# JunkyByte/easy_ViTPose

Measured on AMD Instinct MI355X. Metric: persons_per_sec, higher is better.
Workload: dtype fp16; 1 GPU; ViTPose-B coco K=17, batch 256 x 256x192 crops per GPU (f32 input resident in HBM) -> (y,x,conf) keypoints in HBM; global_batch=256, weights=seeded random init (no checkpoint offline)

## Files before the change

easy_vitpose_amd/build.py:

```python
from __future__ import annotations

import os
import shutil
import subprocess
import sys
from concurrent.futures import ThreadPoolExecutor

HERE = os.path.dirname(os.path.abspath(__file__))
CSRC = os.path.join(HERE, 'csrc')
LIBDIR = os.path.join(HERE, '_lib')
LIB = os.path.join(LIBDIR, 'libvitpose_hip.so')
TOOLS_LIB = os.path.join(LIBDIR, 'libvitpose_hip_tools.so')
SOURCES = ['gemm.hip', 'gemm8.hip', 'gemm8f.hip', 'qkvattn.hip', 'quant8.hip', 'attention.hip', 'elementwise.hip', 'decode.hip', 'boxes.hip', 'fp8_probe.hip',
           'handle.hip', 'forward.hip', 'infer.hip', 'group.hip', 'weights.hip', 'tile_rules.hip', 'debug_taps.hip']
TOOLS_SOURCES = SOURCES + ['probes.hip', 'tools_taps.hip']
HEADERS = ['common.h', 'kernels.h', 'tiles.h', 'dbg_util.h', 'gemm8_common.h', 'mx8.h', 'api_internal.h', 'boxgeom.h', os.path.join('..', '..', 'include', 'vitpose_hip.h'),
           os.path.join('..', '..', 'include', 'vitpose_hip_tools.h')]
FLAGS = ['--offload-arch=gfx950', '-O3', '-std=c++17', '-fPIC', '-fvisibility=hidden',
         '-ffp-contract=fast', '-Wno-unused-result']


def _hipcc() -> str:
    for cand in (shutil.which('hipcc'), '/opt/rocm/bin/hipcc'):
        if cand and os.path.exists(cand):
            return cand
    raise RuntimeError('hipcc not found: the HIP extension cannot be built (no CPU fallback exists)')


def _stale(target: str, deps: "list[str]") -> bool:
    if not os.path.exists(target):
        return True
    t = os.path.getmtime(target)
    return any(os.path.getmtime(d) > t for d in deps)


def build_library(force: bool = False, verbose: bool = False, tools: bool = False) -> str:
    os.makedirs(LIBDIR, exist_ok=True)
    hipcc = _hipcc()
    hdrs = [os.path.normpath(os.path.join(CSRC, h)) for h in HEADERS]
# ... 30 lines not shown
```

easy_vitpose_amd/csrc/api_internal.h:

```cpp
#pragma once
#include <hip/hip_runtime.h>

#include <algorithm>
#include <cmath>
#include <cstdio>
#include <cstdlib>
#include <cstring>
#include <string>
#include <unordered_map>
#include <vector>

#include "../../include/vitpose_hip.h"
#ifdef VP_TOOLS
#include "../../include/vitpose_hip_tools.h"
#endif
#include "kernels.h"
#include "mx8.h"

namespace vpi {

struct Block {
    float *ln1_g, *ln1_b, *ln2_g, *ln2_b;
    uint16_t *w_qkv, *w_proj, *w_fc1, *w_fc2;
    float *b_qkv, *b_proj, *b_fc1, *b_fc2;
    float *s_qkv, *s_fc1;
    uint16_t* w_qkvh = nullptr;
    float *b_qkvh = nullptr, *s_qkvh = nullptr;
    uint8_t *w_qkv8 = nullptr, *w_fc18 = nullptr, *w_fc28 = nullptr, *w_proj8 = nullptr;
    float *ws_qkv = nullptr, *ws_fc1 = nullptr, *ws_fc2 = nullptr, *ws_proj = nullptr;
};

struct Switches {
    int g8_stagger = 0;
    int gemm8_mask = 0x7;
    long g8_min_tiles = 448;
    bool persist_gemm = true;
    int order_mask = 8;
    bool blocked_hid = true;
    bool blocked_qkv = true;
    bool fuse_ln = true;
    bool fuse_qkv_attn = true;
    bool qa_min_set = false;
    long qa_min_tiles = 108;
    long qa80_min_tiles = 192;
    int qa80_group = 8;
    int attn_qsplit = 128;
    int g8_bm192 = 3;
    bool pad_batch = true;
    bool g8_cost_model = true;
    bool deconv_parity_fast = true;
    bool fuse_head = true;
    bool fp8_proj16 = false;
    int graph_max_n = 16;
    bool graph_null = true;
    int caller_stream_max_n = 16;
    bool fold_rule = true;
    int graph_max_n_stats = 8;
    bool splitk_on = true;
    int splitk_force[2][2] = {{0, 0}, {0, 0}};
    int gemm_variant[VP_PROF_COUNT] = {-1, -1, -1, -1, -1, -1, -1, -1, -1, -1, -1};
    int gemm_group_m[VP_PROF_COUNT] = {0};
    int fam_ablate[VP_PROF_COUNT] = {0};
};

}

namespace vpi {
struct MixPlan {
// ... 191 lines not shown
    size_t plane = 0;
    float* stats_out = nullptr;
    const float* rowstat = nullptr;
    const float* ln_s = nullptr;
    const float* ln_part = nullptr;
    int ln_tiles = 0;
    int* tiles_out = nullptr;
};

constexpr int SPLITK_MAX_S = 8, SPLITK_MAX_CROPS = 32;
struct GemmPick { int variant = -1, group_m = 0, persist = 0, stagger = 0, splitk = 1, splitk_variant = 0; };
GemmPick resolve_gemm(const Switches& s, int fam, int epi, int M, int N, int K, bool ln_part = false, size_t splitk_rows = 0,
                      const std::vector<int>* mix_bounds = nullptr);
GemmPick resolve_gemm_fp8(int fam, int epi, int Mp, int N);
enum QkvPath { QKV_GEMM = 0, QKV_ATTN64 = 1, QKV_ATTN80 = 2 };
struct HeadPlan {
    bool fused = false;
    GemmPick deconv1, deconv2, final;
};
struct ChunkPlan {
    int n = 0;
    bool fold1 = false, fold2 = false;
    int qkv_path = QKV_GEMM;
    bool attn_qsplit = false;
    bool proj_fp8 = false;
    GemmPick gemm[VP_PROF_COUNT];
    HeadPlan head;
};
ChunkPlan plan_chunk(const Switches& s, int D, int heads, int max_batch, bool fp8, int n_in, size_t fin_rows, const std::vector<int>* mix_bounds = nullptr);
HeadPlan plan_head(const Switches& s, int D, int nh, size_t fin_rows);

int gemm(vp_ctx* c, int fam, int epi, const GemmPick& pk, const uint16_t* A, const uint16_t* W, const float* bias, void* out,
         const float* aux, int M, int N, int K, int ldo, int Hin = 0, int Win = 0, int Cin = 0, const LnFuse* ln = nullptr);
int gemm_fp8(vp_ctx* c, int fam, int epi, const GemmPick& pk, const uint8_t* A8, const uint8_t* a_scales, const uint8_t* W8, const float* w_scale, const float* bias,
             void* out, uint8_t* out_scales, const float* aux, int M, int N, int K, const LnFuse* ln);
struct FwdOpts {
    bool tokens = false;
    bool mirror = false;
    bool head = true;
    int twin_src = 0;
};
int forward_chunk(vp_ctx* c, const void* d_crops, int fmt, int n_in, const FwdOpts& o = FwdOpts());
int head_chunk(vp_ctx* c, const uint16_t* y, int nh, float* hm, const HeadPlan& hp);
int decode_chunk(vp_ctx* c, const int32_t* d_wh, float* d_out, int n, bool twin);
int chunk_cap(const vp_ctx* c);
int chunk_rows(const vp_ctx* c, int nb);
// ... 5 lines not shown
```

easy_vitpose_amd/csrc/forward.hip:

```cpp
#include "api_internal.h"
#include "tiles.h"

using namespace vpi;

namespace vpi {

static void note_kernel(vp_ctx* c, int fam, const char* desc) {
    if (desc[0] && c->kernel_desc[fam] != desc) c->kernel_desc[fam] = desc;
}

int gemm(vp_ctx* c, int fam, int epi, const GemmPick& pk, const uint16_t* A, const uint16_t* W, const float* bias, void* out,
         const float* aux, int M, int N, int K, int ldo, int Hin, int Win, int Cin, const LnFuse* ln) {
    vp::GemmArgs g{};
    g.A = A; g.W = W; g.bias = bias; g.out = out; g.aux = aux;
    g.M = M; g.N = N; g.K = K; g.ldo = ldo;
    g.Hin = Hin; g.Win = Win; g.Cin = Cin; g.zero = c->zero; g.Kp = c->Kp;
    g.w_rows = (int)pad128((size_t)N);
    g.variant = pk.variant; g.group_m = pk.group_m; g.persist = pk.persist; g.stagger = pk.stagger;
    g.ablate = c->gemm_ablate | c->sw.fam_ablate[fam];
    g.parity_fast = c->sw.deconv_parity_fast;
    if (c->mix_expert && fam == VP_PROF_GEMM_FC2) g.expert = c->mix_expert;
    if (ln) {
        g.a_blocked = ln->a_blocked; g.out_blocked = ln->out_blocked; g.reverse = ln->reverse;
        g.plane = ln->plane; g.stats_out = ln->stats_out; g.rowstat = ln->rowstat; g.ln_s = ln->ln_s;
// ... 126 lines not shown
        };
        const double qkv_attn_flops = 2.0 * M * 3.0 * D * D + 4.0 * 192 * 192 * (double)D * n, qkv_attn_bytes = 2.0 * M * D + 2.0 * 3 * D * (double)D + 2.0 * M * D;
        if ((rc = gemm(c, VP_PROF_GEMM_PATCH, vp::EPI_POS_LN, pk[VP_PROF_GEMM_PATCH], c->hid, c->w_patch, c->b_zero, c->x, c->pos, M, D, 768, D, 0, 0, 0, &prod))) return rc;
        if ((rc = finalize(pl.fold1))) return rc;
        for (int l = 0; l < c->L; ++l) {
            const Block& b = c->blocks[l];
            if (pl.qkv_path == QKV_ATTN80) {
                vp::GemmArgs g80{};
                g80.A = xh; g80.W = b.w_qkvh; g80.bias = b.b_qkvh; g80.ln_s = b.s_qkvh; g80.rowstat = c->rowstat; g80.out = c->y;
                g80.M = M; g80.N = c->heads * 256; g80.K = D; g80.ldo = D; g80.w_rows = c->heads * 256; g80.variant = 18;
                g80.group_m = c->sw.qa80_group;
                g80.attn_scale_log2e = (1.0f / sqrtf(80.0f)) * 1.4426950408889634f;
                g80.ablate = c->gemm_ablate | c->sw.fam_ablate[VP_PROF_GEMM_QKV];
                char desc[192];
                desc[0] = 0;
                g80.desc = desc; g80.desc_cap = (int)sizeof(desc);
                LAUNCH(c, VP_PROF_GEMM_QKV, qkv_attn_flops, qkv_attn_bytes, vp::gemm_launch(c->dtype, vp::EPI_QKV_ATTN, g80, c->stream));
                note_kernel(c, VP_PROF_GEMM_QKV, desc);
            } else if (pl.qkv_path == QKV_ATTN64) {
                vp::QkvAttnArgs qa{};
                qa.x_hi = xh; qa.wh = b.w_qkvh; qa.bh = b.b_qkvh; qa.sh = b.s_qkvh; qa.rowstat = c->rowstat; qa.y = c->y;
                qa.npairs = (n + 1) / 2; qa.ncrops = n; qa.heads = c->heads; qa.D = D;
                qa.scale_log2e = (1.0f / sqrtf(64.0f)) * 1.4426950408889634f;
                char desc[96];
                desc[0] = 0;
                LAUNCH(c, VP_PROF_GEMM_QKV, qkv_attn_flops, qkv_attn_bytes, vp::qkvattn_launch(c->dtype, qa, c->stream, desc, (int)sizeof(desc)));
                note_kernel(c, VP_PROF_GEMM_QKV, desc);
            } else {
                LnFuse cq; cq.rowstat = c->rowstat; cq.ln_s = b.s_qkv; cq.reverse = (c->sw.order_mask & 1) != 0; cq.out_blocked = qkv_blocked;
                if (pl.fold1) { cq.rowstat = nullptr; cq.ln_part = c->ln_part; cq.ln_tiles = D / 64; }
                if ((rc = gemm(c, VP_PROF_GEMM_QKV, vp::EPI_BIAS, pk[VP_PROF_GEMM_QKV], xh, b.w_qkv, b.b_qkv, c->qkv, nullptr, M, 3 * D, D, 3 * D, 0, 0, 0, &cq))) return rc;
                if ((rc = attention(c->y, 8.0 * M * D, nullptr))) return rc;
            }
            LnFuse pp = prod; pp.reverse = (c->sw.order_mask & 2) != 0;
            if ((rc = gemm(c, VP_PROF_GEMM_PROJ, vp::EPI_BIAS_RESID_LN, pk[VP_PROF_GEMM_PROJ], c->y, b.w_proj, b.b_proj, c->x, c->x, M, D, D, D, 0, 0, 0, &pp))) return rc;
            if ((rc = finalize(pl.fold2))) return rc;
            LnFuse c1; c1.rowstat = c->rowstat; c1.ln_s = b.s_fc1; c1.out_blocked = c->sw.blocked_hid; c1.reverse = (c->sw.order_mask & 4) != 0;
            if (pl.fold2) { c1.rowstat = nullptr; c1.ln_part = c->ln_part; c1.ln_tiles = D / 64; }
            if ((rc = gemm(c, VP_PROF_GEMM_FC1, vp::EPI_BIAS_GELU, pk[VP_PROF_GEMM_FC1], xh, b.w_fc1, b.b_fc1, c->hid, nullptr, M, 4 * D, D, 4 * D, 0, 0, 0, &c1))) return rc;
            LnFuse p2 = prod; p2.a_blocked = c->sw.blocked_hid; p2.reverse = (c->sw.order_mask & 8) != 0;
            if ((rc = gemm(c, VP_PROF_GEMM_FC2, vp::EPI_BIAS_RESID_LN, pk[VP_PROF_GEMM_FC2], c->hid, fc2_w(c, b), fc2_b(c, b), c->x, c->x, M, D, 4 * D, D, 0, 0, 0, &p2))) return rc;
            if (l + 1 < c->L && (rc = finalize(pl.fold1))) return rc;
        }
    } else {
    if ((rc = gemm(c, VP_PROF_GEMM_PATCH, vp::EPI_POS, pk[VP_PROF_GEMM_PATCH], c->hid, c->w_patch, c->b_zero, c->x, c->pos, M, D, 768, D))) return rc;
    for (int l = 0; l < c->L; ++l) {
// ... 178 lines not shown
```

easy_vitpose_amd/csrc/handle.hip:

```cpp
#include "api_internal.h"

using namespace vpi;

namespace vpi {

thread_local std::string g_create_error;

int fail(vp_ctx* c, int code, const std::string& msg) {
    if (c) c->err = msg; else g_create_error = msg;
    return code;
}

int need_weights(vp_ctx* c) {
    if (!c) return VP_ERR_INVALID;
    return c->loaded ? (int)VP_OK : fail(c, VP_ERR_STATE, "weights not loaded: call vp_load_weights first");
}

bool slots_busy(const vp_ctx* c) { return c->slots[0].busy || c->slots[1].busy; }

int slots_idle(vp_ctx* c, const char* who) {
    return slots_busy(c) ? fail(c, VP_ERR_STATE, std::string(who) + " with a vp_infer_submit in flight: call vp_infer_wait first") : (int)VP_OK;
}

int quiesce(vp_ctx* c) {
// ... 44 lines not shown
            t += used;
            if (*t == ',') ++t; else break;
        }
    }
#endif
}

void read_switches(Switches& s) {
    auto on = [](const char* name, bool& dst) { if (const char* f = getenv(name)) dst = atoi(f) != 0; };
    auto num = [](const char* name, auto& dst) { if (const char* f = getenv(name)) dst = atol(f); };
    on("VP_FUSE_LN", s.fuse_ln);
    on("VP_PERSIST", s.persist_gemm);
    if (const char* f = getenv("VP_GRAPH")) s.graph_max_n = atoi(f) == 1 ? 16 : atoi(f);
    on("VP_GRAPH_NULL", s.graph_null);
    if (const char* f = getenv("VP_CALLER_STREAM")) s.caller_stream_max_n = atoi(f) == 1 ? 16 : atoi(f);
    on("VP_FUSE_HEAD", s.fuse_head);
    if (const char* f = getenv("VP_FOLD_STATS")) { s.graph_max_n_stats = atoi(f); s.fold_rule = false; }
    on("VP_BLOCKED_QKV", s.blocked_qkv);
    on("VP_FUSE_QKV_ATTN", s.fuse_qkv_attn);
    s.qa_min_set = getenv("VP_QA_MIN_TILES") != nullptr;
    num("VP_QA_MIN_TILES", s.qa_min_tiles);
    num("VP_QA80_MIN_TILES", s.qa80_min_tiles);
    num("VP_QA80_GROUP", s.qa80_group);
    num("VP_ATTN_QSPLIT", s.attn_qsplit);
    on("VP_DECONV_PARITY_FAST", s.deconv_parity_fast);
    on("VP_G8_COST", s.g8_cost_model);
    on("VP_PAD_BATCH", s.pad_batch);
    num("VP_G8_BM192", s.g8_bm192);
    if (const char* f = getenv("VP_SPLITK")) {
        if (!strchr(f, ':')) s.splitk_on = atoi(f) != 0;
        else {
            const char* t = f;
            while (*t) {
                const int which = !strncmp(t, "fc2:", 4) ? 1 : !strncmp(t, "proj:", 5) ? 0 : -1;
                if (which < 0) break;
                t = strchr(t, ':') + 1;
                int S = 0, v = 0, used = 0;
                if (sscanf(t, "%d:%d%n", &S, &v, &used) != 2) break;
                s.splitk_force[which][0] = S; s.splitk_force[which][1] = v;
                t += used;
                if (*t == ',') ++t;
            }
        }
    }
    num("VP_GEMM8", s.gemm8_mask);
    s.fp8_proj16 = getenv("VP_FP8_PROJ16") != nullptr;
// ... 287 lines not shown
```

easy_vitpose_amd/csrc/kernels.h:

```cpp
#pragma once
#include <hip/hip_runtime.h>
#include <stdint.h>

#ifdef VP_TOOLS
#define VP_ABLATE(g) ((g).ablate)
#define VP_STAGGER(g) ((g).stagger)
namespace vp {
hipError_t peak_bench(int kind, double* result);
hipError_t hwid_probe_launch(uint32_t* d_out, int blocks, int threads, int lds_bytes, int spin, hipStream_t s);
}
#else
#define VP_ABLATE(g) 0
#define VP_STAGGER(g) 0
#endif

namespace vp {

enum { DT_F16 = 0, DT_BF16 = 1 };

enum GemmEpi {
    EPI_BIAS = 0,
    EPI_BIAS_GELU = 1,
    EPI_BIAS_RESID = 2,
    EPI_POS = 3,
    EPI_DECONV = 4,
// ... 63 lines not shown
hipError_t ln_finalize_launch(const float* partials, float* rowstat, int M, int tiles, int D, hipStream_t s);
hipError_t splitk_reduce_launch(int dtype, const float* partials, int S, const float* bias, uint16_t* x_hi, size_t plane, float* stats_out, int M, int N,
                                hipStream_t s);

hipError_t fp8_probe_launch(const float* dA, const float* dW, const float* dAs, const float* dWs, uint8_t* dA8, uint8_t* dW8, float* dOut,
                            int M, int N, int K, hipStream_t s);

hipError_t mx_probe_launch(const float* dA, const float* dW, const float* dWs, uint8_t* dA8, uint8_t* dAs, uint8_t* dW8, float* dOut,
                           int M, int N, int K, hipStream_t s);

hipError_t attention_launch(int dtype, const uint16_t* qkv, uint16_t* out, int B, int D, int heads, hipStream_t s, bool qsplit, int qkv_blocked = 0,
                            uint8_t* mx_scales = nullptr);

struct QkvAttnArgs {
    const uint16_t* x_hi;
    const uint16_t* wh;
    const float* bh;
    const float* sh;
    const float* rowstat;
    uint16_t* y;
    int npairs, heads, D;
    int ncrops;
    float scale_log2e;
    int ablate;
};
bool qkvattn_supported(const QkvAttnArgs& a);
hipError_t qkvattn_launch(int dtype, const QkvAttnArgs& a, hipStream_t s, char* desc, int desc_cap);
hipError_t qkv_head_major_launch(const uint16_t* w, const float* b, const float* s, uint16_t* wh, float* bh, float* sh, int D, int K, hipStream_t st);
hipError_t qkv_head_major80_launch(const uint16_t* w, const float* b, const float* s, uint16_t* wh, float* bh, float* sh, int D, int K, int heads, hipStream_t st);

hipError_t layernorm_launch(int dtype, const float* x, const float* gamma, const float* beta,
                            uint16_t* out16, float* out32, int M, int D, hipStream_t s, size_t plane = 0);
hipError_t im2col_launch(int dtype, const void* crops, int input_format, uint16_t* out, int B, hipStream_t s, bool flip = false, int n_src = 0);
hipError_t gather_crops_launch(const void* src, void* dst, const int32_t* idx, int n, size_t crop_bytes, hipStream_t s);
hipError_t flip_merge_launch(float* hm, const float* hm_flipped, const int32_t* partner, int N, int K, int shift, hipStream_t s, int interleaved = 0);
hipError_t im2col_twin_launch(int dtype, const void* crops, int input_format, uint16_t* out, int B, int n_src, hipStream_t s);
void flip_twin_layout(int bo, int n_src, int* src, int* mirror);

struct CropRec {
    const uint8_t* src;
    int64_t pitch;
    int32_t cw, ch, left, top, pw, ph;
};
hipError_t crop_resize_launch(const CropRec* recs, uint8_t* out, int n, hipStream_t s);

constexpr int BOX_FRAMES_PER_LAUNCH = 128;
// ... 32 lines not shown
```

easy_vitpose_amd/csrc/qkvattn.hip:

```cpp
#include <cstdio>
#include <cstdlib>

#include "gemm8_common.h"

namespace vp {

namespace {
struct QA {
    static constexpr int NT = 512;
    static constexpr int XS = 192 * 128;
    static constexpr int W0S = 128 * 128, W1S = 64 * 128;
    static constexpr int OFF_X0 = 0, OFF_X1 = XS, OFF_W0 = 2 * XS, OFF_W1 = 2 * XS + W0S;
    static constexpr int BUF = 2 * XS + W0S + W1S;
    static constexpr int RING = 2 * BUF;
    static constexpr int VSUB = 192 * 32;
    static constexpr int V_BASE = 4 * XS;
    static_assert(6 * XS == RING && BUF <= 3 * XS && BUF + XS <= 4 * XS, "the attention phase reuses exactly the ring; buffer 0 + X0 of buffer 1 inside Q0 K0 Q1 K1");
};

__device__ __forceinline__ u32x2 lds_read_tr16(const char* p) {
    typedef __attribute__((__vector_size__(4 * sizeof(__fp16)))) __fp16 h4;
    typedef __attribute__((address_space(3))) h4* lds_h4;
    const h4 v = __builtin_amdgcn_ds_read_tr16_b64_v4f16((lds_h4)(p));
    return __builtin_bit_cast(u32x2, v);
}
}

template <class T>
__global__ __launch_bounds__(512, 2) void qkvattn_kernel(QkvAttnArgs g) {
    constexpr int QT = 3;
    extern __shared__ __attribute__((aligned(16))) char smem[];
    const int tid = threadIdx.x, lane = tid & 63;
    const int wave = __builtin_amdgcn_readfirstlane(tid >> 6);
    const int wr = wave >> 2, wc = wave & 3;
    const int K = g.D, nk = K >> 6;
    const int ntiles = g.npairs * g.heads;
    const int xcd = blockIdx.x & 7, j0 = blockIdx.x >> 3;
    const int nloc = (gridDim.x >> 3) + (xcd < (int)(gridDim.x & 7) ? 1 : 0);
    const int tq = ntiles >> 3, tr8 = ntiles & 7;
    const int tbase = (xcd < tr8) ? xcd * (tq + 1) : tr8 * (tq + 1) + (xcd - tr8) * tq;
    const int tcnt = tq + (xcd < tr8 ? 1 : 0);
    if (j0 >= tcnt) return;

    const int rip = lane >> 3, pslot = lane & 7;
    const int slog = pslot ^ (((wave & 1) << 2) | (rip >> 1));
    const uint32_t voff = (uint32_t)(rip * K + slog * 8) * 2u;
    const size_t r64 = (size_t)64 * K * 2;
    const char* xb = nullptr;
    const char* wb = nullptr;
    size_t xb1off = 0;
    int pair = 0, head = 0;
    int ipair = 0, ihead = 0;
    auto set_tile = [&](int t) {
        const int tile = tbase + t;
        ipair = tile / g.heads;
        ihead = tile - ipair * g.heads;
        xb = (const char*)(g.x_hi + ((size_t)ipair * 384 + wave * 8) * K);
        xb1off = (2 * ipair + 1 < g.ncrops) ? (size_t)192 * K * 2 : 0;
        wb = (const char*)(g.wh + ((size_t)ihead * 192 + wave * 8) * K);
    };
    auto issue = [&](int which, int B, int kt) {
        char* dst = smem + B * QA::BUF + wave * 1024;
        uint32_t v = voff;
        asm volatile("" : "+v"(v));
        if (which < 2) {
            const char* src = xb + (which ? xb1off : 0) + (size_t)kt * 128 + v;
            glds16(src, dst + which * QA::XS);
            glds16(src + r64, dst + which * QA::XS + 8192);
            glds16(src + 2 * r64, dst + which * QA::XS + 16384);
        } else if (which == 2) {
            const char* src = wb + (size_t)kt * 128 + v;
            glds16(src, dst + QA::OFF_W0);
            glds16(src + r64, dst + QA::OFF_W0 + 8192);
        } else {
            const char* src = wb + 2 * r64 + (size_t)kt * 128 + v;
            glds16(src, dst + QA::OFF_W1);
        }
    };

// ... 61 lines not shown
            for (int j = 0; j < 6; ++j) {
                acc[0][6 + j] = mfma16<T>(fa[0][kk], xs[j][kk], acc[0][6 + j]);
                acc[1][6 + j] = mfma16<T>(fa[1][kk], xs[j][kk], acc[1][6 + j]);
                acc[2][6 + j] = mfma16<T>(fb[kk], xs[j][kk], acc[2][6 + j]);
            }
        __builtin_amdgcn_s_setprio(0);
        bar();
    };
    using M0 = std::integral_constant<int, 0>;
    using M1 = std::integral_constant<int, 1>;
    using M2 = std::integral_constant<int, 2>;
    using M3 = std::integral_constant<int, 3>;
    using B0 = std::integral_constant<int, 0>;
    using B1 = std::integral_constant<int, 1>;
    auto ring_start = [&]() {
        issue(2, 0, 0); issue(0, 0, 0); issue(3, 0, 0); issue(1, 0, 0);
        issue(2, 1, 1); issue(0, 1, 1); issue(3, 1, 1);
        wait_vm<6>();
        bar();
        if (wr) bar();
    };

    int t = j0;
    set_tile(t);
    ring_start();
    for (;;) {
        pair = ipair;
        head = ihead;
        const bool has_next = t + nloc < tcnt;
        bool prefetched = false;
#pragma unroll
        for (int f = 0; f < 3; ++f)
#pragma unroll
            for (int j = 0; j < 12; ++j) acc[f][j] = f32x4{0.f, 0.f, 0.f, 0.f};
        ktile(B0{}, M1{}, 1, 2);
        ktile(B1{}, M0{}, 2, 3);
        for (int kt = 2; kt < nk - 2; kt += 2) {
            if (VP_ABLATE(g) & 4) break;
            ktile(B0{}, M0{}, kt + 1, kt + 2);
            ktile(B1{}, M0{}, kt + 2, kt + 3);
        }
        ktile(B0{}, M2{}, nk - 1, 0);
        ktile(B1{}, M3{}, 0, 0);
        int frow_e = frow, fg_e = fg;
        asm volatile("" : "+v"(frow_e), "+v"(fg_e));
        const int cb = head * 192 + fg_e * 4;
        f32x4 b4[3], s4[3];
        float2 stat[12];
#pragma unroll
        for (int f = 0; f < 3; ++f) {
            const int c = cb + (f < 2 ? wc * 32 + f * 16 : 128 + wc * 16);
            b4[f] = *(const f32x4*)(g.bh + c);
// ... 49 lines not shown
            const size_t b = (size_t)pair * 2 + ((2 * pair + 1 < g.ncrops) ? crop : 0);
#pragma unroll
            for (int t0 = 0; t0 < 3; t0 += QT) {
                u32x4 qf[QT][2];
#pragma unroll
                for (int tq_ = 0; tq_ < QT; ++tq_)
#pragma unroll
                    for (int kk = 0; kk < 2; ++kk) qf[tq_][kk] = *(const u32x4*)(Qs + ((lw * 3 + t0 + tq_) * 16 + fr) * 128 + (((kk * 4 + fg) ^ kswz) << 4));
                f32x4 s[QT][12];
#pragma unroll
                for (int tq_ = 0; tq_ < QT; ++tq_)
#pragma unroll
                    for (int kt = 0; kt < 12; ++kt) s[tq_][kt] = f32x4{0.f, 0.f, 0.f, 0.f};
#pragma unroll
                for (int kt = 0; kt < 12; ++kt)
#pragma unroll
                    for (int kk = 0; kk < 2; ++kk) {
                        const u32x4 kf = *(const u32x4*)(kfrag + kt * 16 * 128 + (((kk * 4 + fg) ^ kswz) << 4));
#pragma unroll
                        for (int tq_ = 0; tq_ < QT; ++tq_) s[tq_][kt] = mfma16<T>(kf, qf[tq_][kk], s[tq_][kt]);
                    }
                __syncthreads();
                if (has_next) {
                    set_tile(t + nloc);
                    issue(2, 0, 0); issue(0, 0, 0); issue(3, 0, 0); issue(1, 0, 0);
                    issue(0, 1, 1);
                    prefetched = true;
                }
                u32x4 pf[QT][6];
                float inv_l[QT];
#pragma unroll
                for (int tq_ = 0; tq_ < QT; ++tq_) {
                    float mx = -3.0e38f;
#pragma unroll
                    for (int kt = 0; kt < 12; ++kt)
#pragma unroll
                        for (int r = 0; r < 4; ++r) mx = fmaxf(mx, s[tq_][kt][r]);
                    mx = fmaxf(mx, __shfl_xor(mx, 16, 64));
                    mx = fmaxf(mx, __shfl_xor(mx, 32, 64));
                    float l = 0.f;
                    const float mb = mx * g.scale_log2e;
#pragma unroll
                    for (int kt = 0; kt < 12; ++kt)
#pragma unroll
                        for (int r = 0; r < 4; ++r) {
                            const float p = softmax_p(s[tq_][kt][r], g.scale_log2e, mb);
                            s[tq_][kt][r] = p;
// ... 31 lines not shown
#pragma unroll
                    for (int tq_ = 0; tq_ < QT; ++tq_) {
                        const int q = (lw * 3 + t0 + tq_) * 16 + fr;
                        uint16_t* dst = g.y + (b * 192 + q) * g.D + head * 64;
                        u32x4 w;
                        w[0] = pack2_nosat<T>(o[0][tq_][0] * inv_l[tq_], o[0][tq_][1] * inv_l[tq_]);
                        w[1] = pack2_nosat<T>(o[0][tq_][2] * inv_l[tq_], o[0][tq_][3] * inv_l[tq_]);
                        w[2] = pack2_nosat<T>(o[1][tq_][0] * inv_l[tq_], o[1][tq_][1] * inv_l[tq_]);
                        w[3] = pack2_nosat<T>(o[1][tq_][2] * inv_l[tq_], o[1][tq_][3] * inv_l[tq_]);
                        *(u32x4*)(dst + dp * 16 + fg * 8) = w;
                    }
                }
            }
        }
        if (!has_next) break;
        t += nloc;
        __syncthreads();
        if (prefetched) {
            issue(2, 1, 1); issue(3, 1, 1);
            wait_vm<6>();
            bar();
            if (wr) bar();
        } else {
            set_tile(t);
            ring_start();
        }
    }
}

__global__ void qkv_head_major_kernel(const uint16_t* __restrict__ w, const float* __restrict__ b, const float* __restrict__ s, uint16_t* __restrict__ wh,
                                      float* __restrict__ bh, float* __restrict__ sh, int D, int K) {
    const int dst = blockIdx.x;
    const int h = dst / 192, r = dst - h * 192;
    int src;
    if (r < 128) {
        const int wc = r >> 5, p = (r >> 4) & 1, rho = r & 15;
        src = p * D + h * 64 + wc * 16 + rho;
    } else {
        src = 2 * D + h * 64 + (r - 128);
    }
    for (int k = threadIdx.x; k < K; k += blockDim.x) wh[(size_t)dst * K + k] = w[(size_t)src * K + k];
    if (threadIdx.x == 0) { bh[dst] = b[src]; sh[dst] = s[src]; }
}

hipError_t qkv_head_major_launch(const uint16_t* w, const float* b, const float* s, uint16_t* wh, float* bh, float* sh, int D, int K, hipStream_t st) {
    if (D % 64) return hipErrorInvalidValue;
    hipLaunchKernelGGL(qkv_head_major_kernel, dim3(3 * D), dim3(256), 0, st, w, b, s, wh, bh, sh, D, K);
// ... 15 lines not shown
    return hipGetLastError();
}

bool qkvattn_supported(const QkvAttnArgs& a) {
    if (a.D % 128 || a.D < 256 || a.heads * 64 != a.D || a.npairs <= 0 || (a.ncrops != 2 * a.npairs && a.ncrops != 2 * a.npairs - 1)) return false;
    if ((size_t)a.npairs * 384 * a.D * 2 >= (1ull << 32)) return false;
    return a.npairs * a.heads >= 8;
}

hipError_t qkvattn_launch(int dtype, const QkvAttnArgs& a, hipStream_t s, char* desc, int desc_cap) {
    if (!qkvattn_supported(a)) return hipErrorInvalidValue;
    const int tiles = a.npairs * a.heads;
    const int grid = tiles < 256 ? tiles : 256;
    static bool attr_done[2][64] = {};
    int dev = 0;
    (void)hipGetDevice(&dev);
    const int di = dtype == DT_F16 ? 0 : 1;
    auto kern = dtype == DT_F16 ? qkvattn_kernel<F16> : qkvattn_kernel<BF16>;
    if (dev < 0 || dev >= 64 || !attr_done[di][dev]) {
        hipError_t e = hipFuncSetAttribute((const void*)kern, hipFuncAttributeMaxDynamicSharedMemorySize, QA::RING);
        if (e != hipSuccess) return e;
        if (dev >= 0 && dev < 64) attr_done[di][dev] = true;
    }
    if (desc) snprintf(desc, desc_cap, "qkvattn_kernel<%s>", dtype == DT_F16 ? "F16" : "BF16");
    hipLaunchKernelGGL(kern, dim3(grid), dim3(QA::NT), QA::RING, s, a);
    return hipGetLastError();
}

}
```

easy_vitpose_amd/csrc/tile_rules.hip:

```cpp
#include "api_internal.h"
#include "tiles.h"

using namespace vpi;

namespace vpi {

struct G8Pick { int variant, bm, bn; long tiles; };
struct Tile2Pick { int variant, group_m; };
using vp::is_gemm8;
struct SplitKPick { int S, variant; };

G8Pick pick_gemm8_tile(int M, int N, bool wide, int bm192_mask, long min_tiles, bool extended) {
    const bool ext = extended && M >= 7680;
    const long t2 = (long)((M + 191) / 192) * ((N + 127) / 128);
    const double cost2 = t2 <= 256 ? 24576.0 : (double)((t2 + 511) / 512) * 49152.0;
    G8Pick pk{0, 0, 0, 0};
    double best = 0.0;
    bool have256 = false;
    for (const vp::Tile8Row& cd : vp::TILES8) {
        if (M % cd.BM || N % cd.BN || (wide && cd.id == 17)) continue;
        if (cd.id == 18 && (!(bm192_mask & (wide ? 2 : 1)) || (!ext && have256))) continue;
        const long t = (long)(M / cd.BM) * (N / cd.BN);
        if (t < 8) continue;
        const long rounds = (t + 255) / 256;
// ... 95 lines not shown
    return (c0 > 0.0 && c1 > 0.0 && c1 < 0.95 * c0) ? n4 : n;
}

int tile_bm(int variant) {
    if (const int bm8 = vp::tile8_bm(variant)) return bm8;
    int bm = 0, bn = 0, slots = 0;
    return tile2_dims(variant, bm, bn, slots) ? bm : 0;
}

bool expert_tile_ok(int bm, const std::vector<int>& bounds) {
    if (bm <= 0) return false;
    for (int b : bounds)
        if (((long)b * 192) % bm) return false;
    return true;
}

int expert_fallback_variant(int M, int N, bool gemm8_ok, int* group_m) {
    constexpr vp::Tile8Row t8 = *vp::find_tile8(18);
    if (gemm8_ok && N % t8.BN == 0 && (long)(M / t8.BM) * (N / t8.BN) >= 448) { *group_m = 2; return t8.id; }
    *group_m = 0;
    return 11;
}

static int gemm8_group_m(int fam) { return fam == VP_PROF_GEMM_QKV ? 4 : fam == VP_PROF_GEMM_FC2 ? 2 : 8; }

GemmPick resolve_gemm(const Switches& s, int fam, int epi, int M, int N, int K, bool ln_part, size_t splitk_rows, const std::vector<int>* mix_bounds) {
    GemmPick p;
    const bool tuned = s.gemm_variant[fam] >= 0;
    const bool wide = epi == vp::EPI_BIAS || epi == vp::EPI_BIAS_GELU;
    const int w_rows = (int)pad128((size_t)N);
    if (tuned) {
        p.variant = s.gemm_variant[fam]; p.group_m = s.gemm_group_m[fam];
    } else {
        const Tile2Pick tp = pick_gemm2_tile(epi, M, N, K);
        p.variant = tp.variant; p.group_m = tp.group_m;
    }
    if (s.persist_gemm && p.variant == 8 && wide && K % 128 == 0 && M % 192 == 0 && N % 128 == 0 && (long)(M / 192) * (N / 128) >= 1024)
        p.persist = 1;
    const int g8bit = fam == VP_PROF_GEMM_FC2 ? 1 : fam == VP_PROF_GEMM_FC1 ? 2 : fam == VP_PROF_GEMM_QKV ? 4 : fam == VP_PROF_GEMM_PROJ ? 8 : 0;
    if (!tuned && (s.gemm8_mask & g8bit) && (wide || epi == vp::EPI_BIAS_RESID_LN)) {
        const G8Pick pk = pick_gemm8_tile(M, N, wide, s.g8_bm192, s.g8_min_tiles, s.g8_cost_model);
        if (pk.variant && vp::gemm8_shape_ok(epi, M, N, K, N, w_rows, pk.bn, pk.bm)) {
            p.variant = pk.variant; p.group_m = gemm8_group_m(fam); p.persist = 0; p.stagger = s.g8_stagger;
        }
    }
    if (epi == vp::EPI_DECONV_FINAL) { p.variant = 3; p.group_m = 0; p.persist = 0; }
// ... 69 lines not shown
    if (!s.fuse_ln) {
        p.gemm[VP_PROF_GEMM_QKV] = gemm(VP_PROF_GEMM_QKV, vp::EPI_BIAS, 3 * D, D, false);
        p.gemm[VP_PROF_GEMM_FC1] = gemm(VP_PROF_GEMM_FC1, vp::EPI_BIAS_GELU, 4 * D, D, false);
        return p;
    }
    const bool fold_stats = n <= s.graph_max_n_stats;
    auto folds = [&](int fam, int epi, int N) {
        if (fold_stats) return true;
        if (!s.fold_rule || n > 64 || s.gemm_variant[fam] >= 0) return false;
        const int v = gemm(fam, epi, N, D, false).variant;
        return vp::tile_folds_stats(v);
    };
    const bool has_qkvh = s.fuse_qkv_attn && (hd == 64 || (heads * 80 == D && D % 128 == 0));
    const bool qkv_can_fold = folds(VP_PROF_GEMM_QKV, vp::EPI_BIAS, 3 * D);
    const long pair_tiles = (long)((n + 1) / 2) * heads;
    const bool want80 = has_qkvh && heads * 80 == D && (long)n * heads >= s.qa80_min_tiles;
    const bool want64 = has_qkvh && heads * 64 == D && pair_tiles >= s.qa_min_tiles && (s.qa_min_set || pair_tiles >= 128 || !qkv_can_fold);
    p.fold1 = fold_stats || (!want80 && !want64 && qkv_can_fold);
    p.fold2 = folds(VP_PROF_GEMM_FC1, vp::EPI_BIAS_GELU, 4 * D);
    vp::QkvAttnArgs qa{};
    qa.npairs = (n + 1) / 2; qa.ncrops = n; qa.heads = heads; qa.D = D;
    if (s.gemm_variant[VP_PROF_GEMM_QKV] < 0 && !p.fold1) {
        if (want80 && vp::gemm8_shape_ok(vp::EPI_QKV_ATTN, M, heads * 256, D, D, heads * 256, 256, 192)) p.qkv_path = QKV_ATTN80;
        else if (want64 && vp::qkvattn_supported(qa)) p.qkv_path = QKV_ATTN64;
    }
    p.gemm[VP_PROF_GEMM_QKV] = gemm(VP_PROF_GEMM_QKV, vp::EPI_BIAS, 3 * D, D, p.fold1);
    p.gemm[VP_PROF_GEMM_FC1] = gemm(VP_PROF_GEMM_FC1, vp::EPI_BIAS_GELU, 4 * D, D, p.fold2);
    return p;
}

}

extern "C" {

VP_API int vp_dbg_expert_tile(int32_t variant, int32_t M, int32_t N, int32_t gemm8_ok, const int32_t* bounds, int32_t n_bounds) {
    if (M <= 0 || N <= 0 || n_bounds < 0 || (n_bounds > 0 && !bounds)) return VP_ERR_INVALID;
    const std::vector<int> b(bounds, bounds + n_bounds);
    if (expert_tile_ok(tile_bm(variant), b)) return variant;
    int gm = 0;
    return expert_fallback_variant(M, N, gemm8_ok != 0, &gm);
}

VP_API int vp_dbg_run_batch(int32_t n, int32_t D, int32_t limit) {
    if (n <= 0 || D <= 0) return VP_ERR_INVALID;
    return pick_run_batch(Switches{}, n, D, limit);
}

// ... 39 lines not shown
```

Before: 25490 persons/s.

## Add configurable tile-walk orders for the fused QKV-attention kernel

Moves the per-XCD tile assignment of the fused QKV+attention kernel into a host-computed walk table passed as kernel arguments. The table supports head-group sweep and XCD-blocked orders meant to improve L2 reuse of weights and activations. The shipped default stays head-fastest unless VP_QA64_GROUP is set, so the default path only picks up extra per-tile index logic and a larger kernel argument struct. An L2 traffic model is included for tuning.

```diff
diff --git a/easy_vitpose_amd/build.py b/easy_vitpose_amd/build.py
--- a/easy_vitpose_amd/build.py
+++ b/easy_vitpose_amd/build.py
@@ -14,7 +14,7 @@
 SOURCES = ['gemm.hip', 'gemm8.hip', 'gemm8f.hip', 'qkvattn.hip', 'quant8.hip', 'attention.hip', 'elementwise.hip', 'decode.hip', 'boxes.hip', 'fp8_probe.hip',
            'handle.hip', 'forward.hip', 'infer.hip', 'group.hip', 'weights.hip', 'tile_rules.hip', 'debug_taps.hip']
 TOOLS_SOURCES = SOURCES + ['probes.hip', 'tools_taps.hip']
-HEADERS = ['common.h', 'kernels.h', 'tiles.h', 'dbg_util.h', 'gemm8_common.h', 'mx8.h', 'api_internal.h', 'boxgeom.h', os.path.join('..', '..', 'include', 'vitpose_hip.h'),
+HEADERS = ['common.h', 'kernels.h', 'tiles.h', 'dbg_util.h', 'gemm8_common.h', 'qkvattn_order.h', 'mx8.h', 'api_internal.h', 'boxgeom.h', os.path.join('..', '..', 'include', 'vitpose_hip.h'),
            os.path.join('..', '..', 'include', 'vitpose_hip_tools.h')]
 FLAGS = ['--offload-arch=gfx950', '-O3', '-std=c++17', '-fPIC', '-fvisibility=hidden',
          '-ffp-contract=fast', '-Wno-unused-result']
diff --git a/easy_vitpose_amd/csrc/api_internal.h b/easy_vitpose_amd/csrc/api_internal.h
--- a/easy_vitpose_amd/csrc/api_internal.h
+++ b/easy_vitpose_amd/csrc/api_internal.h
@@ -44,6 +44,8 @@
     long qa_min_tiles = 108;
     long qa80_min_tiles = 192;
     int qa80_group = 8;
+    bool qa64_set = false;
+    int qa64_group = 0;
     int attn_qsplit = 128;
     int g8_bm192 = 3;
     bool pad_batch = true;
@@ -281,6 +283,7 @@
     int n = 0;
     bool fold1 = false, fold2 = false;
     int qkv_path = QKV_GEMM;
+    int qa_order = 0, qa_hg = 0;
     bool attn_qsplit = false;
     bool proj_fp8 = false;
     GemmPick gemm[VP_PROF_COUNT];
diff --git a/easy_vitpose_amd/csrc/forward.hip b/easy_vitpose_amd/csrc/forward.hip
--- a/easy_vitpose_amd/csrc/forward.hip
+++ b/easy_vitpose_amd/csrc/forward.hip
@@ -172,6 +172,7 @@
                 qa.x_hi = xh; qa.wh = b.w_qkvh; qa.bh = b.b_qkvh; qa.sh = b.s_qkvh; qa.rowstat = c->rowstat; qa.y = c->y;
                 qa.npairs = (n + 1) / 2; qa.ncrops = n; qa.heads = c->heads; qa.D = D;
                 qa.scale_log2e = (1.0f / sqrtf(64.0f)) * 1.4426950408889634f;
+                qa.order = pl.qa_order; qa.hg = pl.qa_hg;
                 char desc[96];
                 desc[0] = 0;
                 LAUNCH(c, VP_PROF_GEMM_QKV, qkv_attn_flops, qkv_attn_bytes, vp::qkvattn_launch(c->dtype, qa, c->stream, desc, (int)sizeof(desc)));
diff --git a/easy_vitpose_amd/csrc/handle.hip b/easy_vitpose_amd/csrc/handle.hip
--- a/easy_vitpose_amd/csrc/handle.hip
+++ b/easy_vitpose_amd/csrc/handle.hip
@@ -90,6 +90,8 @@
     num("VP_QA_MIN_TILES", s.qa_min_tiles);
     num("VP_QA80_MIN_TILES", s.qa80_min_tiles);
     num("VP_QA80_GROUP", s.qa80_group);
+    s.qa64_set = getenv("VP_QA64_GROUP") != nullptr;
+    num("VP_QA64_GROUP", s.qa64_group);
     num("VP_ATTN_QSPLIT", s.attn_qsplit);
     on("VP_DECONV_PARITY_FAST", s.deconv_parity_fast);
     on("VP_G8_COST", s.g8_cost_model);
diff --git a/easy_vitpose_amd/csrc/kernels.h b/easy_vitpose_amd/csrc/kernels.h
--- a/easy_vitpose_amd/csrc/kernels.h
+++ b/easy_vitpose_amd/csrc/kernels.h
@@ -1,6 +1,7 @@
 #pragma once
 #include <hip/hip_runtime.h>
 #include <stdint.h>
+#include "qkvattn_order.h"
 
 #ifdef VP_TOOLS
 #define VP_ABLATE(g) ((g).ablate)
@@ -110,6 +111,8 @@
     int npairs, heads, D;
     int ncrops;
     float scale_log2e;
+    int order, hg;
+    QaWalk walk[8];
     int ablate;
 };
 bool qkvattn_supported(const QkvAttnArgs& a);
diff --git a/easy_vitpose_amd/csrc/qkvattn.hip b/easy_vitpose_amd/csrc/qkvattn.hip
--- a/easy_vitpose_amd/csrc/qkvattn.hip
+++ b/easy_vitpose_amd/csrc/qkvattn.hip
@@ -34,12 +34,9 @@
     const int wave = __builtin_amdgcn_readfirstlane(tid >> 6);
     const int wr = wave >> 2, wc = wave & 3;
     const int K = g.D, nk = K >> 6;
-    const int ntiles = g.npairs * g.heads;
     const int xcd = blockIdx.x & 7, j0 = blockIdx.x >> 3;
-    const int nloc = (gridDim.x >> 3) + (xcd < (int)(gridDim.x & 7) ? 1 : 0);
-    const int tq = ntiles >> 3, tr8 = ntiles & 7;
-    const int tbase = (xcd < tr8) ? xcd * (tq + 1) : tr8 * (tq + 1) + (xcd - tr8) * tq;
-    const int tcnt = tq + (xcd < tr8 ? 1 : 0);
+    const int nloc = qa_xcd_workgroups(xcd, (int)gridDim.x);
+    const int tcnt = g.walk[xcd].tcnt;
     if (j0 >= tcnt) return;
 
     const int rip = lane >> 3, pslot = lane & 7;
@@ -51,10 +48,14 @@
     size_t xb1off = 0;
     int pair = 0, head = 0;
     int ipair = 0, ihead = 0;
-    auto set_tile = [&](int t) {
-        const int tile = tbase + t;
-        ipair = tile / g.heads;
-        ihead = tile - ipair * g.heads;
+    auto locate = [&](int t, int& p, int& h) {
+        int x = blockIdx.x & 7;
+        asm volatile("" : "+s"(x));
+        qa_walk_tile(g.walk[x], t, p, h);
+    };
+    auto set_tile = [&](int p, int h) {
+        ipair = p;
+        ihead = h;
         xb = (const char*)(g.x_hi + ((size_t)ipair * 384 + wave * 8) * K);
         xb1off = (2 * ipair + 1 < g.ncrops) ? (size_t)192 * K * 2 : 0;
         wb = (const char*)(g.wh + ((size_t)ihead * 192 + wave * 8) * K);
@@ -162,12 +163,15 @@
     };
 
     int t = j0;
-    set_tile(t);
+    int npair = 0, nhead = 0;
+    locate(t, npair, nhead);
+    set_tile(npair, nhead);
     ring_start();
     for (;;) {
         pair = ipair;
         head = ihead;
         const bool has_next = t + nloc < tcnt;
+        if (has_next) locate(t + nloc, npair, nhead);
         bool prefetched = false;
 #pragma unroll
         for (int f = 0; f < 3; ++f)
@@ -263,7 +267,7 @@
                     }
                 __syncthreads();
                 if (has_next) {
-                    set_tile(t + nloc);
+                    set_tile(npair, nhead);
                     issue(2, 0, 0); issue(0, 0, 0); issue(3, 0, 0); issue(1, 0, 0);
                     issue(0, 1, 1);
                     prefetched = true;
@@ -341,7 +345,7 @@
             bar();
             if (wr) bar();
         } else {
-            set_tile(t);
+            set_tile(npair, nhead);
             ring_start();
         }
     }
@@ -403,8 +407,14 @@
         if (e != hipSuccess) return e;
         if (dev >= 0 && dev < 64) attr_done[di][dev] = true;
     }
-    if (desc) snprintf(desc, desc_cap, "qkvattn_kernel<%s>", dtype == DT_F16 ? "F16" : "BF16");
-    hipLaunchKernelGGL(kern, dim3(grid), dim3(QA::NT), QA::RING, s, a);
+    if (desc) {
+        const QaOrder o = qa_order_norm(a.heads, a.order, a.hg);
+        if (o.order == QA_HEAD_FASTEST) snprintf(desc, desc_cap, "qkvattn_kernel<%s>", dtype == DT_F16 ? "F16" : "BF16");
+        else snprintf(desc, desc_cap, "qkvattn_kernel<%s> order %d hg %d", dtype == DT_F16 ? "F16" : "BF16", o.order, o.hg);
+    }
+    QkvAttnArgs k = a;
+    for (int x = 0; x < 8; ++x) k.walk[x] = qa_walk(x, a.npairs, a.heads, a.order, a.hg);
+    hipLaunchKernelGGL(kern, dim3(grid), dim3(QA::NT), QA::RING, s, k);
     return hipGetLastError();
 }
 
diff --git a/easy_vitpose_amd/csrc/qkvattn_order.h b/easy_vitpose_amd/csrc/qkvattn_order.h
--- /dev/null
+++ b/easy_vitpose_amd/csrc/qkvattn_order.h
@@ -0,0 +1,149 @@
+#pragma once
+#include <algorithm>
+#include <vector>
+
+#if defined(__HIPCC__)
+#define VP_QA_HD __host__ __device__ inline
+#else
+#define VP_QA_HD inline
+#endif
+
+namespace vp {
+
+enum { QA_HEAD_FASTEST = 0, QA_GROUP_SWEEP = 1, QA_XCD_BLOCK = 2 };
+
+struct QaOrder { int order, hg; };
+
+VP_QA_HD QaOrder qa_order_norm(int heads, int order, int hg) {
+    if (order != QA_GROUP_SWEEP && order != QA_XCD_BLOCK) return {QA_HEAD_FASTEST, heads};
+    if (hg < 1 || hg >= heads) return {QA_HEAD_FASTEST, heads};
+    const int ng = (heads + hg - 1) / hg;
+    if (order == QA_XCD_BLOCK && (ng > 8 || 8 % ng)) order = QA_GROUP_SWEEP;
+    return {order, hg};
+}
+
+VP_QA_HD void qa_split(int n, int parts, int i, int& first, int& count) {
+    const int q = n / parts, r = n - q * parts;
+    first = i < r ? i * (q + 1) : r * (q + 1) + (i - r) * q;
+    count = q + (i < r ? 1 : 0);
+}
+
+VP_QA_HD int qa_xcd_workgroups(int xcd, int grid) { return (grid >> 3) + (xcd < (grid & 7) ? 1 : 0); }
+
+struct QaWalk {
+    int tcnt;
+    int order, heads, hg;
+    int lo;
+    int pf, hf, pl, hl;
+    int p0, h0, nh;
+};
+
+VP_QA_HD QaWalk qa_walk(int xcd, int npairs, int heads, int order, int hg) {
+    const QaOrder o = qa_order_norm(heads, order, hg);
+    QaWalk w{};
+    w.order = o.order; w.heads = heads; w.hg = o.hg;
+    if (o.order == QA_XCD_BLOCK) {
+        const int ng = (heads + o.hg - 1) / o.hg;
+        const int gi = xcd % ng, ri = xcd / ng;
+        int np = 0;
+        qa_split(npairs, 8 / ng, ri, w.p0, np);
+        w.h0 = gi * o.hg;
+        w.nh = heads - w.h0 < o.hg ? heads - w.h0 : o.hg;
+        w.tcnt = np * w.nh;
+    } else {
+        qa_split(npairs * heads, 8, xcd, w.lo, w.tcnt);
+        const int last = w.lo + (w.tcnt > 0 ? w.tcnt - 1 : 0);
+        w.pf = w.lo / heads; w.hf = w.lo - w.pf * heads;
+        w.pl = last / heads; w.hl = last - w.pl * heads;
+    }
+    return w;
+}
+
+VP_QA_HD void qa_walk_tile(const QaWalk& w, int q, int& pair, int& head) {
+    if (w.order == QA_XCD_BLOCK) {
+        const int dp = q / w.nh;
+        pair = w.p0 + dp;
+        head = w.h0 + (q - dp * w.nh);
+        return;
+    }
+    if (w.order == QA_HEAD_FASTEST) {
+        const int tile = w.lo + q;
+        pair = tile / w.heads;
+        head = tile - pair * w.heads;
+        return;
+    }
+    const int pf = w.pf, hf = w.hf, pl = w.pl, hl = w.hl;
+    for (int a = 0; a < w.heads; a += w.hg) {
+        const int b = a + w.hg < w.heads ? a + w.hg : w.heads;
+        int fa = a > hf ? a : hf, fb = b;
+        if (pf == pl && hl + 1 < fb) fb = hl + 1;
+        const int c0 = fb > fa ? fb - fa : 0;
+        if (q < c0) { pair = pf; head = fa + q; return; }
+        q -= c0;
+        if (pl > pf) {
+            const int mid = (pl - pf - 1) * (b - a);
+            if (q < mid) {
+                const int dp = q / (b - a);
+                pair = pf + 1 + dp;
+                head = a + (q - dp * (b - a));
+                return;
+            }
+            q -= mid;
+            const int lb = hl + 1 < b ? hl + 1 : b;
+            const int c1 = lb > a ? lb - a : 0;
+            if (q < c1) { pair = pl; head = a + q; return; }
+            q -= c1;
+        }
+    }
+    pair = pl; head = hl;
+}
+
+VP_QA_HD bool qa_tile(int xcd, int q, int npairs, int heads, int order, int hg, int& pair, int& head) {
+    const QaWalk w = qa_walk(xcd, npairs, heads, order, hg);
+    if (q < 0 || q >= w.tcnt) return false;
+    qa_walk_tile(w, q, pair, head);
+    return true;
+}
+
+struct QaTraffic { double x_bytes, w_bytes; };
+
+inline bool qa_round_resident(int nheads_round, int npairs_round, int D, double l2_bytes = 4.0 * 1024 * 1024) {
+    const double wp = 192.0 * D * 2, xp = 384.0 * D * 2;
+    return nheads_round * wp + 0.5 * npairs_round * xp <= l2_bytes;
+}
+
+inline QaTraffic qa_traffic(int npairs, int heads, int D, int grid, int order, int hg) {
+    const double wp = 192.0 * D * 2, xp = 384.0 * D * 2;
+    QaTraffic t{0.0, 0.0};
+    if (npairs <= 0 || heads <= 0 || heads > 64) return t;
+    std::vector<char> pairs_prev(npairs), pairs_now(npairs);
+    for (int xcd = 0; xcd < 8; ++xcd) {
+        const QaWalk w = qa_walk(xcd, npairs, heads, order, hg);
+        const int nloc = qa_xcd_workgroups(xcd, grid);
+        if (nloc <= 0) continue;
+        unsigned long long heads_prev = 0;
+        bool x_kept = false;
+        std::fill(pairs_prev.begin(), pairs_prev.end(), 0);
+        for (int r0 = 0; r0 < w.tcnt; r0 += nloc) {
+            unsigned long long heads_now = 0;
+            int nh = 0, np = 0, np_new = 0;
+            std::fill(pairs_now.begin(), pairs_now.end(), 0);
+            for (int q = r0; q < w.tcnt && q < r0 + nloc; ++q) {
+                int p = 0, h = 0;
+                qa_walk_tile(w, q, p, h);
+                if (!(heads_now >> h & 1)) { heads_now |= 1ull << h; ++nh; }
+                if (!pairs_now[p]) { pairs_now[p] = 1; ++np; np_new += !(x_kept && pairs_prev[p]); }
+            }
+            const bool resident = qa_round_resident(nh, np, D);
+            int nh_new = 0;
+            for (int h = 0; h < heads; ++h) nh_new += (heads_now >> h & 1) && !(resident && (heads_prev >> h & 1));
+            t.x_bytes += np_new * xp;
+            t.w_bytes += nh_new * wp;
+            heads_prev = heads_now;
+            x_kept = np * xp <= 4.0 * 1024 * 1024;
+            pairs_prev.swap(pairs_now);
+        }
+    }
+    return t;
+}
+}
diff --git a/easy_vitpose_amd/csrc/tile_rules.hip b/easy_vitpose_amd/csrc/tile_rules.hip
--- a/easy_vitpose_amd/csrc/tile_rules.hip
+++ b/easy_vitpose_amd/csrc/tile_rules.hip
@@ -1,5 +1,6 @@
 #include "api_internal.h"
 #include "tiles.h"
+#include "qkvattn_order.h"
 
 using namespace vpi;
 
@@ -141,6 +142,18 @@
     return 11;
 }
 
+constexpr int QA64_SHIP_ORDER = vp::QA_HEAD_FASTEST;
+static vp::QaOrder pick_qa64_order(const Switches& s, int heads, int D, long tiles) {
+    if (s.qa64_set) {
+        const int v = s.qa64_group;
+        return vp::qa_order_norm(heads, v > 0 ? vp::QA_GROUP_SWEEP : v < 0 ? vp::QA_XCD_BLOCK : vp::QA_HEAD_FASTEST, v < 0 ? -v : v);
+    }
+    if (QA64_SHIP_ORDER == vp::QA_HEAD_FASTEST || tiles < 256) return vp::qa_order_norm(heads, vp::QA_HEAD_FASTEST, heads);
+    for (int hg = heads; hg >= 2; --hg)
+        if (heads % hg == 0 && vp::qa_round_resident(hg, (32 + hg - 1) / hg + 1, D)) return vp::qa_order_norm(heads, QA64_SHIP_ORDER, hg);
+    return vp::qa_order_norm(heads, vp::QA_HEAD_FASTEST, heads);
+}
+
 static int gemm8_group_m(int fam) { return fam == VP_PROF_GEMM_QKV ? 4 : fam == VP_PROF_GEMM_FC2 ? 2 : 8; }
 
 GemmPick resolve_gemm(const Switches& s, int fam, int epi, int M, int N, int K, bool ln_part, size_t splitk_rows, const std::vector<int>* mix_bounds) {
@@ -256,7 +269,11 @@
     qa.npairs = (n + 1) / 2; qa.ncrops = n; qa.heads = heads; qa.D = D;
     if (s.gemm_variant[VP_PROF_GEMM_QKV] < 0 && !p.fold1) {
         if (want80 && vp::gemm8_shape_ok(vp::EPI_QKV_ATTN, M, heads * 256, D, D, heads * 256, 256, 192)) p.qkv_path = QKV_ATTN80;
-        else if (want64 && vp::qkvattn_supported(qa)) p.qkv_path = QKV_ATTN64;
+        else if (want64 && vp::qkvattn_supported(qa)) {
+            p.qkv_path = QKV_ATTN64;
+            const vp::QaOrder o = pick_qa64_order(s, heads, D, pair_tiles);
+            p.qa_order = o.order; p.qa_hg = o.hg;
+        }
     }
     p.gemm[VP_PROF_GEMM_QKV] = gemm(VP_PROF_GEMM_QKV, vp::EPI_BIAS, 3 * D, D, p.fold1);
     p.gemm[VP_PROF_GEMM_FC1] = gemm(VP_PROF_GEMM_FC1, vp::EPI_BIAS_GELU, 4 * D, D, p.fold2);
```

Result: no change. 25490 persons/s, median of 2 (-0.0%).
